# alshai/rowbowt

Hardware: AMD Instinct MI355X
Metric: reads/s (100 bp, count+locate) (higher is better)
Workload: dtype u32/u64

## Files before the change

### rowbowt_amd/csrc/k_runs.hip

```cpp
#include <type_traits>

#include "rbg_runs2_device.hpp"
#include "rbg_jump.h"

namespace rbg {
namespace {

struct PackedBits {
    const uint4 *__restrict__ cp;
    uint4 w;
    uint32_t widx, navail;
    uint64_t sr;
    __device__ __forceinline__ uint32_t next_word() {
        if (widx == 4) { w = *cp++; widx = 0; }
        const uint32_t v = w.x;
        w.x = w.y; w.y = w.z; w.z = w.w;
        ++widx;
        return v;
    }
    __device__ __forceinline__ uint32_t take(uint32_t nb) {
        if (navail < nb) { sr |= static_cast<uint64_t>(next_word()) << navail; navail += 32; }
        const uint32_t v = static_cast<uint32_t>(sr & ((uint64_t(1) << nb) - 1));
        sr >>= nb;
        navail -= nb;
        return v;
    }
};

struct JumpLoad {
    const uint4 *__restrict__ tab;
    __device__ __forceinline__ void operator()(uint64_t b, uint32_t s, uint32_t kw[4], uint32_t vw[4]) const {
        const uint4 *sl = tab + (4 * b + 2 * s);
        const uint4 k = sl[0], v = sl[1];
        kw[0] = k.x; kw[1] = k.y; kw[2] = k.z; kw[3] = k.w;
        vw[0] = v.x; vw[1] = v.y; vw[2] = v.z; vw[3] = v.w;
    }
};

template <typename P, bool TOEHOLD, bool PACKED = false, bool STATS = false, bool GLDS = false, bool STAGE = false>
__global__ __launch_bounds__(512, STATS ? 2 : 4) void k_find_range_runs(const DevIndex ix, const void *__restrict__ src_a,
                                                        const void *__restrict__ src_b, const uint64_t N,
                                                        uint64_t *__restrict__ lo_out, uint64_t *__restrict__ hi_out,
                                                        uint64_t *__restrict__ ss_out, unsigned long long *__restrict__ stats,
                                                        const uint32_t *__restrict__ sel, const uint32_t *__restrict__ nsel) {
    const uint64_t Neff = sel ? static_cast<uint64_t>(*nsel) : N;
    const uint8_t *__restrict__ seqs = static_cast<const uint8_t *>(src_a);
    const uint64_t *__restrict__ off = static_cast<const uint64_t *>(src_b);
    const uint4 *__restrict__ chunks = static_cast<const uint4 *>(src_a);
    const uint2 *__restrict__ meta = static_cast<const uint2 *>(src_b);
    __shared__ uint8_t s_lut[256];
    __shared__ uint8_t s_lut2[256];
    __shared__ uint8_t s_mslot[4];
    __shared__ __align__(16) unsigned char s_tile[GLDS ? 8 * kTileBytes : 16];
    __shared__ uint32_t s_codes[STAGE ? 8 * kStageWords * 64 : 1];
    for (int t = threadIdx.x; t < 256; t += blockDim.x) {
        s_lut[t] = ix.lut[t];
        s_lut2[t] = ix.nmajor ? ix.lut2[t] : 0xFFu;
    }
    RBG_RUN_SEARCH2_SHARED;
    const RunSearch2<P> S2 = stage_run_search2<P>(ix, s_tab_first, s_ent2, s_dir2, s_rec2, s_dyn);
    const uint32_t *tab_first = s_tab_first;
    lds_byte *tile = (lds_byte *)s_tile + (GLDS ? (threadIdx.x >> 6) * kTileBytes : 0u);
    if (PACKED || STAGE) {
        for (int t = threadIdx.x; t < 256; t += blockDim.x)
            if (s_lut2[t] != 0xFFu) s_mslot[s_lut2[t] & 3u] = s_lut[t];
        __syncthreads();
    }
    const uint32_t D = ix.run_ksteps, DMASK = ix.run_depth_mask | 1u;
    const uint32_t M = ix.nmajor;
    const uint32_t lane = threadIdx.x & (kWave - 1);
    lds_u32 *codes = (lds_u32 *)s_codes + (STAGE ? (threadIdx.x >> 6) * (kStageWords * 64u) + lane : 0u);
    const StageTab stage_tab{ix.stage_code[0], ix.stage_code[1], ix.stage_byte[0], ix.stage_byte[1], ix.stage_shift};
    const bool stage_on = STAGE && ix.stage_ok != 0 && M == 4;

    unsigned long long c_occ = 0, c_reads = 0;
    uint32_t c_matched = 0;
    unsigned long long st[kStatSearchN] = {0, 0, 0, 0, 0, 0, 0, 0};
    const uint64_t stride = static_cast<uint64_t>(gridDim.x) * blockDim.x;
    const uint64_t wave_first = static_cast<uint64_t>(blockIdx.x) * blockDim.x + (threadIdx.x & ~(kWave - 1));
    for (uint64_t base = wave_first; base < Neff; base += stride) {
        bool valid = base + lane < Neff;
        const uint64_t i = (sel && valid) ? static_cast<uint64_t>(sel[base + lane]) : base + lane;
        uint64_t beg = 0, p = 0;
        PackedBits bs{chunks, make_uint4(0, 0, 0, 0), 4u, 0u, 0ull};
        if (PACKED) {
            if (valid) {
                const uint2 mt = meta[i];
                if (mt.y & 0x80000000u) valid = false;
                else { p = mt.y; bs.cp = chunks + mt.x; }
            }
        } else if (valid) { beg = off[i]; p = off[i + 1]; }
        bool staged = false;
        if constexpr (STAGE && !PACKED) {
            if (stage_on && __ballot(valid && p - beg > kStageCap) == 0) {
                uint32_t nch = 0;
                const bool bad = valid && stage_read(reinterpret_cast<const uint4 *>(seqs), beg, p, stage_tab, codes, nch);
                if (STATS) st[kStChunks] += nch;
                staged = __ballot(bad) == 0;
                if (staged) { p -= beg; beg = 0; }
                else if (STATS) st[kStChunks] -= nch;
            }
        }
        auto walk = [&](auto staged_tag) __attribute__((always_inline)) {
            constexpr bool STAGED = decltype(staged_tag)::value;
            const uint64_t p_end = p;
            uint64_t p_min = p;
            const uint32_t m32 = static_cast<uint32_t>(p);
            uint64_t lo = 0, hi = ix.n - 1;
            uint64_t k = TOEHOLD ? ix.last_run_sample : 0;
            bool alive = valid;
            bool pend = false;
            uint32_t pend_d = 0, pend_rec = 0;
            uint64_t pend_e = 0;
            ByteCursor rd{reinterpret_cast<const uint4 *>(seqs), ~uint64_t(0), make_uint4(0, 0, 0, 0)};
            bool jumped = false;
            if constexpr (STAGED && sizeof(P) == 4) {
                if (valid && ix.jump && m32 >= ix.jump_k) {
                    JumpKey key{{codes[0], codes[64], codes[128], codes[192]}};
                    jump_key_mask(key, ix.jump_k);
                    uint32_t v[3] = {0, 0, 0}, nbk = 0;
                    if (jump_probe(JumpLoad{static_cast<const uint4 *>(ix.jump)}, ix.jump_buckets, key, v, nbk)) {
                        lo = v[0]; hi = v[1];
                        if (TOEHOLD) k = v[2] == 0xFFFFFFFFu ? ~uint64_t(0) : static_cast<uint64_t>(v[2]);
                        p -= ix.jump_k;
                        jumped = true;
                        if (STATS) st[kStSymbols] += ix.jump_k;
                    }
                    if (STATS) st[kStFtab] += nbk;
                }
            }
            if (!jumped && valid && ix.ftab_k && p - beg >= ix.ftab_k) {
                uint64_t idx = 0;
                bool all_major = true;
                PackedBits probe = bs;
                if constexpr (STAGED) {
                    const uint32_t w0 = codes[0];
                    idx = ix.ftab_k >= 16u ? w0 : (w0 & ((1u << (2u * ix.ftab_k)) - 1u));
                } else if (PACKED) {
                    idx = probe.take(2 * ix.ftab_k);
                } else {
                    uint64_t pw = 1;
                    for (uint32_t t = 1; t <= ix.ftab_k; ++t) {
                        const uint32_t mm = s_lut2[rd.at(p - t)];
                        all_major = all_major && mm != 0xFFu;
                        idx += (mm & 3u) * pw;
                        pw *= M;
                    }
                }
                uint64_t flo, fhi2, fk;
                if (STATS) { if (!STAGED) p_min = p - ix.ftab_k; if (all_major) st[kStFtab] += 1; }
                if (all_major && ftab_lookup<P>(ix, idx, flo, fhi2, fk)) {
                    if (PACKED) bs = probe;
                    lo = flo; hi = fhi2;
                    if (TOEHOLD) k = fk;
                    p -= ix.ftab_k;
                    if (STATS) st[kStSymbols] += ix.ftab_k;
                    if (hi < lo) { alive = false; p = beg; }
                }
            }
            struct Pick { uint32_t d, adv, rec; bool ok; };
            auto pick_at = [&](const uint64_t pp) __attribute__((always_inline)) -> Pick {
                Pick s{0u, 1u, 0u, true};
                if constexpr (STAGED) {
                    s.adv = pp < D ? static_cast<uint32_t>(pp) : D;
                    s.adv = 32u - static_cast<uint32_t>(__clz(DMASK & ((2u << (s.adv - 1)) - 1u)));
                    const uint32_t t0 = m32 - static_cast<uint32_t>(pp);
                    const lds_u32 *cw = codes + (t0 >> 4) * 64u;
                    const uint32_t v = __builtin_amdgcn_alignbit(cw[64], cw[0], (t0 & 15u) * 2u) & ((1u << (2u * s.adv)) - 1u);
                    s.rec = run_record(tab_first, s.adv, s.adv == 1 ? static_cast<uint32_t>(s_mslot[v]) : v);
                    s.d = s.adv - 1;
                } else if (PACKED) {
                    s.adv = pp < D ? static_cast<uint32_t>(pp) : D;
                    s.adv = 32u - static_cast<uint32_t>(__clz(DMASK & ((2u << (s.adv - 1)) - 1u)));
                    const uint32_t v = bs.take(2 * s.adv);
                    s.rec = run_record(tab_first, s.adv, s.adv == 1 ? static_cast<uint32_t>(s_mslot[v]) : v);
                    s.d = s.adv - 1;
                } else {
                    const uint64_t q = pp - 1;
                    const uint32_t c = rd.at(q);
                    if (STATS && q < p_min) p_min = q;
                    const uint32_t m0 = s_lut2[c];
                    uint32_t acc = m0;
                    if (m0 != 0xFFu) {
                        uint32_t pw = M, run_acc = m0;
    #pragma unroll 1
                        for (uint32_t t = 1; t < static_cast<uint32_t>(kMaxRunDepth); ++t) {
                            if (t >= D || q < beg + t) break;
                            const uint32_t mm = s_lut2[rd.at(q - t)];
                            if (STATS && q - t < p_min) p_min = q - t;
                            if (mm == 0xFFu) break;
                            run_acc += mm * pw;
                            pw *= M;
                            if ((DMASK >> t) & 1u) { s.adv = t + 1; acc = run_acc; }
                        }
                    }
                    if (s.adv == 1) {
                        const uint32_t slot = s_lut[c];
                        if (slot == 0xFFu || slot >= static_cast<uint32_t>(kLdsSyms)) s.ok = false;
                        else s.rec = run_record(tab_first, 1u, slot);
                    } else {
                        s.d = s.adv - 1;
                        s.rec = run_record(tab_first, s.adv, acc);
                    }
                }
                return s;
            };
            constexpr bool AHEAD = !PACKED || STAGED;
            Pick cur{0u, 1u, 0u, false};
            RunHot Rcur{0, 0};
            if (AHEAD && alive && p > beg) {
                cur = pick_at(p);
                if (cur.ok) Rcur = load_run_tab<P>(S2, cur.d, cur.rec);
            }
            while (__ballot(alive && p > beg)) {
                bool stepping = alive && p > beg;
                if (!AHEAD && stepping) {
                    cur = pick_at(p);
                    if (cur.ok) Rcur = load_run_tab<P>(S2, cur.d, cur.rec);
                }
                if (stepping && !cur.ok) { alive = false; stepping = false; }
                const uint32_t d = cur.d, adv = cur.adv, rec = cur.rec;
                const RunHot R = Rcur;
                const uint64_t p_next = p - adv;
                if (AHEAD && stepping && p_next > beg) {
                    cur = pick_at(p_next);
                    if (cur.ok) Rcur = load_run_tab<P>(S2, cur.d, cur.rec);
                }
                RunStep r;
                lane_lf2_quad<P, STATS, false, GLDS>(S2, stepping, d, rec, R, lo, hi + 1, r, st, tile);
                if (stepping) {
                    if (STATS) st[kStSymbols] += adv;
                    const uint64_t c_inside = r.c_upto - r.c_before;
                    if (c_inside == 0) {
                        alive = false;
                    } else {
                        if (TOEHOLD) {
                            if (r.inside) k = k - adv;
                            else { pend = true; pend_d = d; pend_rec = rec; pend_e = r.samp_e; k = 0; }
                        }
                        lo = r.F + r.c_before;
                        hi = lo + c_inside - 1;
                        p = p_next;
                    }
                }
            }
            if (TOEHOLD && alive && pend) {
                k += run_step_sample2<P>(ix, S2, pend_d, pend_rec, pend_e);
                if (STATS) st[kStResample] += 1;
            }
            if (STATS && !PACKED && !STAGED && p_end > p_min) st[kStChunks] += ((p_end - 1) >> 4) - (p_min >> 4) + 1;
            if (STATS && PACKED && valid) st[kStChunks] += (p_end + 63) >> 6;
            if (!alive) { lo = 1; hi = 0; k = 0; }
            if (valid) {
                lo_out[i] = lo;
                hi_out[i] = hi;
                if (TOEHOLD) ss_out[i] = k;
                c_reads += 1;
                if (alive) { c_matched += 1; c_occ += hi - lo + 1; }
            }
        };
        if (STAGE && staged) walk(std::integral_constant<bool, STAGE>{}); else walk(std::false_type{});
    }
    c_reads = wave_sum(c_reads);
    const unsigned long long w_matched = wave_sum(static_cast<unsigned long long>(c_matched));
    c_occ = wave_sum(c_occ);
    if (lane == 0 && c_reads) {
        atomicAdd(&ix.counters[0], c_reads);
        if (w_matched) atomicAdd(&ix.counters[1], w_matched);
        if (c_occ) atomicAdd(&ix.counters[2], c_occ);
    }
    if (STATS) {
#pragma unroll
        for (int t = 0; t < kStatSearchN; ++t) {
            const unsigned long long v = wave_sum(st[t]);
            if (lane == 0 && v) atomicAdd(&stats[t], v);
        }
    }
}

template <typename P> struct ChunkR { static constexpr int v = 8; };
__device__ __forceinline__ uint64_t locus_toehold_r(const DevIndex &ix, const uint64_t key, const uint64_t *__restrict__ k, const uint64_t i) {
    if (key == ~uint64_t(0)) return k[i];
    const uint32_t low = ix.order_lowbits, db = ix.order_dbits;
    const uint64_t doc = (key >> low) & ((uint64_t(1) << db) - 1u);
    return ix.order_docs[doc] + (((key >> (db + low)) << low) | (key & ((uint64_t(1) << low) - 1u)));
}

template <typename P, typename OUT = uint64_t, bool STATS = false, bool SUB = false, bool HI8 = false>
__global__ __launch_bounds__(256, 4) void k_locate_fill_runs2(const DevIndex ix, const uint64_t *__restrict__ lo,
                                                          const uint64_t *__restrict__ hi, const uint64_t *__restrict__ k,
                                                          const uint64_t N, const uint64_t max_hits,
                                                          const uint64_t *__restrict__ loc_off, OUT *__restrict__ locs,
                                                          const uint64_t *__restrict__ sub, const uint32_t *__restrict__ order,
                                                          const uint64_t *__restrict__ skeys, unsigned long long *__restrict__ stats) {
    constexpr int kChunkR = ChunkR<P>::v;
    constexpr bool RING = true;
    using Stage = ChainStage<P, kChunkR, SUB, RING, HI8>;
    __shared__ Stage S;
    const uint64_t out_elem0 = reinterpret_cast<uintptr_t>(locs) / sizeof(OUT);
    const int wv = threadIdx.x >> 6, lane = threadIdx.x & (kWave - 1);
    unsigned long long c_locs = 0;
    unsigned long long st_phi = 0, st_ent = 0, st_chains = 0;
    const uint64_t n = ix.n;
    const uint64_t stride = static_cast<uint64_t>(gridDim.x) * blockDim.x;
    for (uint64_t base = static_cast<uint64_t>(blockIdx.x) * blockDim.x + wv * kWave; base < N; base += stride) {
        const uint64_t j = base + lane;
        uint64_t i = j;
        if (order && j < N) i = order[j];
        uint64_t occ = 0, k1 = 0, dst = 0;
        if (i < N && j < N) {
            dst = loc_off[i];
            if (skeys) {
                if (ix.order_docs) k1 = locus_toehold_r(ix, skeys[j], k, i);
                else if (sizeof(P) == 4) { const uint32_t k32 = reinterpret_cast<const uint32_t *>(skeys)[j]; k1 = k32 == 0xFFFFFFFFu ? k[i] : k32; }
                else k1 = skeys[j];
                occ = loc_off[i + 1] - dst;
            } else {
                const uint64_t l = lo[i], h = hi[i];
                occ = h >= l ? h - l + 1 : 0;
                if (occ > max_hits) occ = max_hits;
                k1 = k[i];
            }
        }
        const uint64_t minus = (SUB && i < N && j < N) ? sub[i] : 0;
        const uint32_t a = (RING && occ) ? static_cast<uint32_t>((out_elem0 + dst) & static_cast<uint64_t>(kChunkR - 1)) : 0u;
        S.dst[wv][lane] = dst - a;
        if (SUB) S.minus[wv][lane] = minus;
        const bool off_text = Stage::kSentinel && k1 >= n;
        if (off_text && occ) locs[dst] = static_cast<OUT>(k1 - minus);
        c_locs += occ;
        if (STATS && occ) st_chains += 1;
        uint64_t wmax = occ + a;
#pragma unroll
        for (int o = kWave / 2; o > 0; o >>= 1) {
            const uint64_t other = __shfl_xor(wmax, o, kWave);
            wmax = other > wmax ? other : wmax;
        }
        for (uint64_t t0 = 0; t0 < wmax; t0 += kChunkR) {
            const uint32_t cnt = chain_round_count<kChunkR>(occ, t0);
            S.bounds[wv][lane] = chain_window_bounds<kChunkR>(occ, a, t0);
#pragma unroll 1
            for (int e = 0; e < kChunkR; ++e) {
                const bool mine = static_cast<uint32_t>(e) < cnt;
                if (mine && (e || t0)) {
                    uint64_t s;
                    if (k1 >= n) {
                        s = (ix.phi_last_base + (k1 - ix.phi_last_pos)) % n;
                    } else {
                        bool found;
                        uint64_t val;
                        uint32_t ents, rounds;
                        lane_phi<P>(ix, k1, found, val, ents, rounds);
                        if (STATS) { st_phi += 1; st_ent += ents + 7u * rounds; }
                        s = found ? val : ix.phi_last_base + k1 + 1;
                        if (s >= n) s -= n;
                    }
                    k1 = s;
                }
                if (mine) chain_put(S, wv, lane, a + static_cast<uint32_t>(t0) + e, k1, e == 0 && t0 == 0 && off_text);
            }
            wave_lds_sync();
            chain_flush(S, wv, lane, t0, locs);
            wave_lds_sync();
        }
        wave_lds_sync();
    }
    c_locs = wave_sum(c_locs);
    if (lane == 0 && c_locs) atomicAdd(&ix.counters[3], c_locs);
    if (STATS) {
        st_phi = wave_sum(st_phi);
        st_ent = wave_sum(st_ent);
        st_chains = wave_sum(st_chains);
        if (lane == 0) {
            if (st_phi) atomicAdd(&stats[kLsPhiSteps], st_phi);
            if (st_ent) atomicAdd(&stats[kLsPhiOvf], st_ent);
            if (st_chains) atomicAdd(&stats[kLsChains], st_chains);
            if (c_locs) atomicAdd(&stats[kLsLocs], c_locs);
        }
    }
}

}

int launch_find_range_runs_impl(const DevIndex &ix, const LaunchCfg &cfg, const void *src_a, const void *src_b, uint64_t N,
                                uint64_t *lo, uint64_t *hi, uint64_t *ssamp, void *stream, bool packed, unsigned long long *stats,
                                const uint32_t *sel = nullptr, const uint32_t *nsel = nullptr) {
    if (N == 0) return 0;
    hipStream_t st = static_cast<hipStream_t>(stream);
    const size_t lds = run_search2_lds(ix);
    static const bool glds = [] { const char *e = std::getenv("RBG_REC_FETCH"); return !(e && std::strcmp(e, "quad") == 0); }();
    static const bool stage = [] { const char *e = std::getenv("RBG_STAGE_READS"); return !(e && e[0] == '0'); }();
    LaunchCfg c = cfg;
    c.block_threads = 512;
    c.max_blocks = cfg.max_blocks > 0 ? std::max(1, cfg.max_blocks / 2) : 256 * 16;
    const dim3 grid(sel ? std::min(grid_for(c, N), 256) : grid_for(c, N)), block(512);
#define RBG_LAUNCH_FRR1(PT, TOE, PK, STS, GL, SG)                                                      \
    do {                                                                                               \
        auto kern = k_find_range_runs<PT, TOE, PK, STS, GL, SG>;                                       \
        raise_lds(kern, lds, (GL ? 8 * kTileBytes : 0) + (SG ? 8 * kStageWaveBytes : 0));             \
        hipLaunchKernelGGL(kern, grid, block, lds, st, ix, src_a, src_b, N, lo, hi, ssamp, stats, sel, nsel);     \
    } while (0)
#define RBG_LAUNCH_FRR(PT, TOE, PK, STS)                                                               \
    do {                                                                                               \
        if (glds && stage && !PK && !sel) RBG_LAUNCH_FRR1(PT, TOE, false, STS, true, true);            \
        else if (glds) RBG_LAUNCH_FRR1(PT, TOE, PK, STS, true, false);                                 \
        else RBG_LAUNCH_FRR1(PT, TOE, PK, STS, false, false);                                          \
    } while (0)
#define RBG_LAUNCH_FRR2(PT, TOE)                                                                       \
    do {                                                                                               \
        if (stats) { if (packed) return static_cast<int>(hipErrorNotSupported); RBG_LAUNCH_FRR(PT, TOE, false, true); } \
        else if (packed) RBG_LAUNCH_FRR(PT, TOE, true, false);                                         \
        else RBG_LAUNCH_FRR(PT, TOE, false, false);                                                    \
    } while (0)
    if (ix.pos_bytes == 4) {
        if (ssamp) RBG_LAUNCH_FRR2(uint32_t, true); else RBG_LAUNCH_FRR2(uint32_t, false);
    } else {
        if (ssamp) RBG_LAUNCH_FRR2(uint64_t, true); else RBG_LAUNCH_FRR2(uint64_t, false);
    }
#undef RBG_LAUNCH_FRR2
#undef RBG_LAUNCH_FRR
#undef RBG_LAUNCH_FRR1
    return static_cast<int>(hipGetLastError());
}

// ... 47 lines not shown
```

### rowbowt_amd/csrc/rbg_jump.h

```cpp
#pragma once

#include <cstdint>

#if defined(__HIPCC__)
#define RBG_JUMP_HD __host__ __device__ __forceinline__
#else
#define RBG_JUMP_HD inline
#endif

namespace rbg {

constexpr uint32_t kJumpMaxK = 64;
constexpr uint32_t kJumpMinK = 16;
constexpr uint32_t kJumpSlotWords = 8;
constexpr uint32_t kJumpBucketBytes = 64;
constexpr uint32_t kJumpEmptyTag = 0, kJumpFullTag = 1;
constexpr uint32_t kJumpDefaultK = 60;
constexpr uint64_t kJumpAutoMinBytes = uint64_t(256) << 20;

struct JumpKey {
    uint32_t w[4];
};

RBG_JUMP_HD void jump_key_mask(JumpKey &key, uint32_t K) {
    for (uint32_t i = 0; i < 4; ++i) {
        const uint32_t lo_sym = 16u * i;
        const uint32_t keep = K <= lo_sym ? 0u : (K - lo_sym >= 16u ? 16u : K - lo_sym);
        key.w[i] = keep == 16u ? key.w[i] : (key.w[i] & ((1u << (2u * keep)) - 1u));
    }
}

RBG_JUMP_HD void jump_key_set(JumpKey &key, uint32_t t, uint32_t c) {
    key.w[t >> 4] |= (c & 3u) << (2u * (t & 15u));
}

RBG_JUMP_HD uint64_t jump_hash(const JumpKey &key) {
    const uint64_t a = key.w[0] | (static_cast<uint64_t>(key.w[1]) << 32);
    const uint64_t b = key.w[2] | (static_cast<uint64_t>(key.w[3]) << 32);
    uint64_t h = (a * 0x9E3779B97F4A7C15ull) ^ ((b + 0x632BE59BD9B4E019ull) * 0xC2B2AE3D27D4EB4Full);
    h ^= h >> 29;
    h *= 0xBF58476D1CE4E5B9ull;
    h ^= h >> 32;
    return h;
}

RBG_JUMP_HD uint64_t jump_home(uint64_t h, uint64_t nb) {
    return ((h >> 32) * nb) >> 32;
}

template <typename Load>
RBG_JUMP_HD bool jump_probe(const Load &load, uint64_t nb, const JumpKey &key, uint32_t v[3], uint32_t &buckets) {
    uint64_t b = jump_home(jump_hash(key), nb);
    for (uint64_t step = 0; step < nb; ++step) {
        ++buckets;
        for (uint32_t s = 0; s < 2; ++s) {
            uint32_t kw[4], vw[4];
            load(b, s, kw, vw);
            if (vw[3] == kJumpEmptyTag) return false;
            if (kw[0] == key.w[0] && kw[1] == key.w[1] && kw[2] == key.w[2] && kw[3] == key.w[3]) {
                v[0] = vw[0]; v[1] = vw[1]; v[2] = vw[2];
                return true;
            }
        }
        b = b + 1 == nb ? 0 : b + 1;
    }
    return false;
}

inline uint64_t jump_buckets_for(uint64_t keys) { return keys ? keys : 1; }

}
```

### rowbowt_amd/csrc/rbg_runs2_device.hpp

```cpp
#pragma once

#include "rbg_runs_device.hpp"

namespace rbg {
namespace {

constexpr int kRunUniAt = 12;
constexpr uint32_t kLaneMaxZ = 15;
constexpr uint32_t kLanePhiMaxZ = 8;

template <typename P>
struct RunSearch2 {
    const uint64_t *hot;
    const uint64_t *ghot;
    const DevRunTab2 *gtab;
    const uint32_t *tab_first;
    const void *const *ent;
    const void *const *dir;
    const void *const *rec;
    const void *rec_any;
    uint32_t fill;
};

#define RBG_RUN_SEARCH2_SHARED                                            \
// ... 119 lines not shown
            A.feed(g, w0.x - a_lo, w0.y);
            A.feed(g + 1u, w0.z - a_lo, w0.w);
            A.feed(g + 2u, w1.x - a_lo, w1.y);
            A.feed(g + 3u, w1.z - a_lo, w1.w);
            if (B) {
                B->feed(g, w0.x - a_lo, w0.y);
                B->feed(g + 1u, w0.z - a_lo, w0.w);
                B->feed(g + 2u, w1.x - a_lo, w1.y);
                B->feed(g + 3u, w1.z - a_lo, w1.w);
            }
        }
        return;
    }
    u32x4a8 w[4], v[4];
#pragma unroll
    for (int j = 0; j < 4; ++j) {
        const uint32_t gj = 2u * j < zw ? 2u * j : zw;
        w[j] = *reinterpret_cast<const RBG_GLOBAL u32x4a8 *>(base + static_cast<uint64_t>(gj) * 8u);
    }
    const bool more = zw >= 8u;
    if (more) {
#pragma unroll
        for (int j = 0; j < 4; ++j) {
            const uint32_t gj = 8u + 2u * j < zw ? 8u + 2u * j : zw;
            v[j] = *reinterpret_cast<const RBG_GLOBAL u32x4a8 *>(base + static_cast<uint64_t>(gj) * 8u);
        }
    }
#pragma unroll
    for (int j = 0; j < 4; ++j) {
        A.feed(2u * j, w[j].x - a_lo, w[j].y);
        A.feed(2u * j + 1u, w[j].z - a_lo, w[j].w);
        if (B) {
            B->feed(2u * j, w[j].x - a_lo, w[j].y);
            B->feed(2u * j + 1u, w[j].z - a_lo, w[j].w);
        }
    }
    if (more) {
#pragma unroll
        for (int j = 0; j < 4; ++j) {
            A.feed(8u + 2u * j, v[j].x - a_lo, v[j].y);
            A.feed(8u + 2u * j + 1u, v[j].z - a_lo, v[j].w);
            if (B) {
                B->feed(8u + 2u * j, v[j].x - a_lo, v[j].y);
                B->feed(8u + 2u * j + 1u, v[j].z - a_lo, v[j].w);
            }
        }
    }
}

constexpr uint32_t kRecScanZ = 7u;
constexpr uint32_t kRecScanZ2 = 15u;
struct LaneRank {
    uint32_t c = 0, lo32 = 0, p = 0, z = 0;
    bool inside = false, pending = false;
    uint32_t qa = 0, a_lo = 0;
};
__device__ __forceinline__ uint32_t sub_sat(const uint32_t a, const uint32_t b) { return __builtin_elementwise_sub_sat(a, b); }
struct LaneRec {
    uint32_t w[16];
    __device__ __forceinline__ void load(const void *__restrict__ recs, const uint64_t at) {
        const RBG_GLOBAL u32x4 *p = as_global<u32x4>(static_cast<const void *>(static_cast<const char *>(recs) + at * 64u));
        const u32x4 a = p[0], b = p[1], c = p[2], d = p[3];
        w[0] = a.x; w[1] = a.y; w[2] = a.z; w[3] = a.w; w[4] = b.x; w[5] = b.y; w[6] = b.z; w[7] = b.w;
        w[8] = c.x; w[9] = c.y; w[10] = c.z; w[11] = c.w; w[12] = d.x; w[13] = d.y; w[14] = d.z; w[15] = d.w;
    }
    __device__ __forceinline__ bool compact() const { return (w[2] & kRec2Compact) != 0; }
    __device__ __forceinline__ void pivots(const uint32_t a_lo, const uint32_t qa, LaneRank &out) const {
        out.qa = qa; out.a_lo = a_lo;
        const uint32_t z = w[3], stride = (z + 12u) / 13u;
        uint32_t m = 0;
#pragma unroll
        for (uint32_t j = 0; j < kRec2Pivots; ++j) m += ((j + 1u) * stride < z && w[4 + j] - a_lo < qa) ? 1u : 0u;
        const uint32_t adv = m * stride;
        out.p = w[0] + adv;
        out.z = (z - adv) < stride ? (z - adv) : stride;
        out.pending = true;
    }
    template <bool NEED_C>
    __device__ __forceinline__ void rank1(const uint32_t sh, const uint32_t a_lo, const uint32_t qa, const uint32_t o, LaneRank &out) const {
        out.qa = qa; out.a_lo = a_lo; out.p = w[0]; out.pending = false;
        const uint32_t mask = ~(~0u << (sh & 31u));
        const uint32_t s0 = w[4] - a_lo, d0 = qa - s0, om1 = o - 1u;
        const bool b0 = (w[2] & 15u) != 0u && s0 < qa;
        uint32_t add = b0 ? (d0 < w[5] ? d0 : w[5]) : 0u, c = b0 ? 1u : 0u;
        bool ins = b0 && d0 <= w[5];
#pragma unroll
        for (uint32_t k = 0; k < kRec2CompactIn; ++k) {
            const uint32_t v = w[6 + k], off = v & mask, len = v >> (sh & 31u);
            const uint32_t d = sub_sat(o, off);
            add += d < len ? d : len;
            if (NEED_C) { c += off < o ? 1u : 0u; ins = ins || (om1 - off) < len; }
        }
        out.c = NEED_C ? c : 1u; out.lo32 = w[3] + add; out.inside = ins;
    }
    __device__ __forceinline__ void rank2(const uint32_t sh, const uint32_t a_lo, const uint32_t qa0, const uint32_t o0, const uint32_t qa1, const uint32_t o1,
                                          LaneRank &A, LaneRank &B) const {
        A.qa = qa0; A.a_lo = a_lo; A.p = w[0]; A.pending = false;
        B.qa = qa1; B.a_lo = a_lo; B.p = w[0]; B.pending = false;
        const uint32_t mask = ~(~0u << (sh & 31u));
        const uint32_t s0 = w[4] - a_lo, l0 = w[5], da = qa0 - s0, db = qa1 - s0, om1 = o1 - 1u;
        const bool have = (w[2] & 15u) != 0u, ba = have && s0 < qa0, bb = have && s0 < qa1;
        uint32_t add_a = ba ? (da < l0 ? da : l0) : 0u, add_b = bb ? (db < l0 ? db : l0) : 0u, c = bb ? 1u : 0u;
        bool ins = bb && db <= l0;
#pragma unroll
        for (uint32_t k = 0; k < kRec2CompactIn; ++k) {
            const uint32_t v = w[6 + k], off = v & mask, len = v >> (sh & 31u);
            const uint32_t ea = sub_sat(o0, off), eb = sub_sat(o1, off);
            add_a += ea < len ? ea : len;
            add_b += eb < len ? eb : len;
            c += off < o1 ? 1u : 0u;
            ins = ins || (om1 - off) < len;
        }
        A.c = 1u;
        A.lo32 = w[3] + add_a; A.inside = false;
        B.c = c; B.lo32 = w[3] + add_b; B.inside = ins;
    }
};

template <typename P, bool WIDE = true>
__device__ __forceinline__ void lane_finish(const RunSearch2<P> &S, const uint32_t d, const uint32_t rec, LaneRank &A, LaneRank *B, uint32_t &rounds, uint32_t &ents) {
    const bool pb = B && B->pending;
    if (!(A.pending || pb)) return;
    const char *__restrict__ tent = static_cast<const char *>(S.ent[d]) + run_first<P>(S, rec) * 8u;
    constexpr uint32_t kMaxZ = WIDE ? kRecScanZ2 : kRecScanZ;
    if (A.pending && A.z > kMaxZ) lane_narrow(tent, A.a_lo, A.qa, A.p, A.z, kMaxZ, 8u, rounds);
    if (pb && B->z > kMaxZ) lane_narrow(tent, B->a_lo, B->qa, B->p, B->z, kMaxZ, 8u, rounds);
    u32x4a8 wa[4], wb[4];
    if (A.pending) {
        const RBG_GLOBAL char *base = as_global<char>(static_cast<const void *>(tent)) + static_cast<uint64_t>(A.p) * 8u;
#pragma unroll
        for (int j = 0; j < 4; ++j) wa[j] = *reinterpret_cast<const RBG_GLOBAL u32x4a8 *>(base + static_cast<uint64_t>(2u * j < A.z ? 2u * j : A.z) * 8u);
    }
    if (pb) {
        const RBG_GLOBAL char *base = as_global<char>(static_cast<const void *>(tent)) + static_cast<uint64_t>(B->p) * 8u;
#pragma unroll
        for (int j = 0; j < 4; ++j) wb[j] = *reinterpret_cast<const RBG_GLOBAL u32x4a8 *>(base + static_cast<uint64_t>(2u * j < B->z ? 2u * j : B->z) * 8u);
    }
    auto take = [&](LaneRank &R, const u32x4a8 (&w)[4]) {
        LaneQ Q;
        Q.qa = R.qa; Q.zlim = R.z;
#pragma unroll
        for (int j = 0; j < 4; ++j) {
            Q.feed(2u * j, w[j].x - R.a_lo, w[j].y);
            Q.feed(2u * j + 1u, w[j].z - R.a_lo, w[j].w);
        }
        if (WIDE && R.z > kRecScanZ && Q.pb) {
            const RBG_GLOBAL char *base = as_global<char>(static_cast<const void *>(tent)) + static_cast<uint64_t>(R.p) * 8u;
            u32x4a8 v[4];
#pragma unroll
            for (int j = 0; j < 4; ++j) v[j] = *reinterpret_cast<const RBG_GLOBAL u32x4a8 *>(base + static_cast<uint64_t>(8u + 2u * j < R.z ? 8u + 2u * j : R.z) * 8u);
#pragma unroll
            for (int j = 0; j < 4; ++j) {
                Q.feed(8u + 2u * j, v[j].x - R.a_lo, v[j].y);
                Q.feed(8u + 2u * j + 1u, v[j].z - R.a_lo, v[j].w);
            }
            ents += 8u;
        }
        R.c = Q.c;
        const uint32_t dd = Q.qa - Q.ks, len = Q.kn - Q.kc;
        R.lo32 = Q.c ? Q.kc + (dd < len ? dd : len) : Q.fc;
        R.inside = Q.c != 0u && dd <= len;
        ents += (R.z < 8u ? R.z + 1u : 8u);
    };
    if (A.pending) take(A, wa);
    if (pb) take(*B, wb);
}


template <typename P, bool STATS = false, bool LEAN = false>
__device__ __forceinline__ void lane_lf2_tab(const RunSearch2<P> &S, const uint32_t d, const uint32_t rec, const RunHot &R, const uint64_t q0, const uint64_t q1, RunStep &out,
                                             unsigned long long *st = nullptr) {
    constexpr bool W = sizeof(P) == 8;
    out.F = 0;
    const uint32_t sh = R.dir_shift;
    const uint64_t b0 = pos_bucket<P>(q0, sh), b1 = pos_bucket<P>(q1, sh);
    if (const void *__restrict__ recs = S.rec[d]) {
        const uint32_t al0 = W ? pos_bucket_base32(q0, sh) - (1u << S.fill) : 0u;
        const uint32_t al1 = W ? pos_bucket_base32(q1, sh) - (1u << S.fill) : 0u;
        const uint32_t qa0 = static_cast<uint32_t>(q0) - al0, qa1 = static_cast<uint32_t>(q1) - al1;
        const uint32_t o0 = pos_bucket_offset(q0, sh), o1 = pos_bucket_offset(q1, sh);
        LaneRank A, B;
        uint32_t h0, h1;
        uint32_t rounds = 0, ents = 0;
        LaneRec r0;
        r0.load(recs, R.dir_off + b0);
        h0 = h1 = r0.w[1];
        if (b1 == b0) {
            if (r0.compact()) r0.rank2(sh, al0, qa0, o0, qa1, o1, A, B);
            else { r0.pivots(al0, qa0, A); r0.pivots(al1, qa1, B); }
            lane_finish<P, !LEAN>(S, d, rec, A, &B, rounds, ents);
        } else if constexpr (LEAN) {
            if (r0.compact()) r0.template rank1<false>(sh, al0, qa0, o0, A); else r0.pivots(al0, qa0, A);
            lane_finish<P, !LEAN>(S, d, rec, A, nullptr, rounds, ents);
            r0.load(recs, R.dir_off + b1);
            h1 = r0.w[1];
            if (r0.compact()) r0.template rank1<true>(sh, al1, qa1, o1, B); else r0.pivots(al1, qa1, B);
            lane_finish<P, !LEAN>(S, d, rec, B, nullptr, rounds, ents);
        } else {
            LaneRec r1;
            r1.load(recs, R.dir_off + b1);
            h1 = r1.w[1];
            if (r0.compact()) r0.template rank1<false>(sh, al0, qa0, o0, A); else r0.pivots(al0, qa0, A);
            if (r1.compact()) r1.template rank1<true>(sh, al1, qa1, o1, B); else r1.pivots(al1, qa1, B);
            lane_finish<P, !LEAN>(S, d, rec, A, &B, rounds, ents);
        }
        if (STATS) { st[kStSlots] += b1 != b0 ? 2 : 1; st[kStSearch] += rounds; st[kStDense] += ents; st[kStSteps] += 1; }
        const uint64_t y0 = static_cast<uint64_t>(h0) << 31, y1 = static_cast<uint64_t>(h1) << 31;
        out.c_before = W ? y0 + static_cast<uint32_t>(A.lo32 - static_cast<uint32_t>(y0)) : A.lo32;
        out.c_upto = W ? y1 + static_cast<uint32_t>(B.lo32 - static_cast<uint32_t>(y1)) : B.lo32;
        out.inside = B.c != 0 && B.inside;
        out.samp_e = static_cast<uint64_t>(B.p) + B.c - 1u;
        return;
    }
    const char *__restrict__ tent = static_cast<const char *>(S.ent[d]) + run_first<P>(S, rec) * 8u;
    const void *__restrict__ dir = S.dir[d];
    uint32_t a0, h0, e0, a1, h1, e1;
    load_dir2<P>(dir, R.dir_off + b0, a0, h0, e0);
    a1 = a0; h1 = h0; e1 = e0;
    if (b1 != b0) load_dir2<P>(dir, R.dir_off + b1, a1, h1, e1);
    if (STATS) st[kStSlots] += b1 != b0 ? 2 : 1;
    uint32_t p0 = a0 ? a0 - 1u : 0u, z0 = e0 - p0;
    uint32_t p1 = a1 ? a1 - 1u : 0u, z1 = e1 - p1;
    const uint32_t al0 = W ? pos_bucket_base32(q0, sh) - (1u << S.fill) : 0u;
    const uint32_t al1 = W ? pos_bucket_base32(q1, sh) - (1u << S.fill) : 0u;
    const uint32_t qa0 = static_cast<uint32_t>(q0) - al0, qa1 = static_cast<uint32_t>(q1) - al1;
    uint32_t rounds = 0;
    if (z0 > kLaneMaxZ) lane_narrow(tent, al0, qa0, p0, z0, kLaneMaxZ, 8u, rounds);
    if (z1 > kLaneMaxZ) lane_narrow(tent, al1, qa1, p1, z1, kLaneMaxZ, 8u, rounds);
    if (STATS) st[kStSearch] += rounds;
    const bool shared = p1 + z1 <= p0 + kLaneMaxZ && (!W || b1 - b0 <= 1u);
    LaneQ A, B;
    A.qa = qa0; A.zlim = z0;
    if (shared) {
        B.qa = static_cast<uint32_t>(q1) - al0; B.zlim = p1 + z1 - p0;
        const uint32_t zw = B.zlim > z0 ? B.zlim : z0;
        lane_scan<LEAN>(tent, p0, zw, al0, A, &B);
        if (STATS) st[kStDense] += zw + 1u;
        p1 = p0;
    } else {
        B.qa = qa1; B.zlim = z1;
        lane_scan<LEAN>(tent, p0, z0, al0, A, nullptr);
        lane_scan<LEAN>(tent, p1, z1, al1, B, nullptr);
        if (STATS) st[kStDense] += z0 + z1 + 2u;
    }
    bool inside = false;
    uint32_t lo32a = A.fc, lo32b = B.fc;
    if (A.c) {
        const uint32_t dd = A.qa - A.ks, len = A.kn - A.kc;
        lo32a = A.kc + (dd < len ? dd : len);
    }
    if (B.c) {
        const uint32_t dd = B.qa - B.ks, len = B.kn - B.kc;
        lo32b = B.kc + (dd < len ? dd : len);
        inside = dd <= len;
    }
    const uint64_t y0 = static_cast<uint64_t>(h0) << 31, y1 = static_cast<uint64_t>(h1) << 31;
    out.c_before = W ? y0 + static_cast<uint32_t>(lo32a - static_cast<uint32_t>(y0)) : lo32a;
    out.c_upto = W ? y1 + static_cast<uint32_t>(lo32b - static_cast<uint32_t>(y1)) : lo32b;
    out.inside = inside;
    out.samp_e = static_cast<uint64_t>(p1) + B.c - 1u;
    if (STATS) st[kStSteps] += 1;
}

template <typename P, bool STATS = false, bool LEAN = false>
__device__ __forceinline__ void lane_lf2(const RunSearch2<P> &S, const uint32_t d, const uint32_t rec, const uint64_t q0, const uint64_t q1, RunStep &out,
                                         unsigned long long *st = nullptr) {
    const RunHot R = load_run_tab<P>(S, d, rec);
    lane_lf2_tab<P, STATS, LEAN>(S, d, rec, R, q0, q1, out, st);
}

__device__ __forceinline__ uint32_t quad_xor1(const uint32_t v) { return static_cast<uint32_t>(__builtin_amdgcn_mov_dpp(static_cast<int>(v), 0xB1, 0xF, 0xF, true)); }
__device__ __forceinline__ uint32_t quad_xor2(const uint32_t v) { return static_cast<uint32_t>(__builtin_amdgcn_mov_dpp(static_cast<int>(v), 0x4E, 0xF, 0xF, true)); }
template <int C>
__device__ __forceinline__ uint32_t quad_bcast(const uint32_t v) { return static_cast<uint32_t>(__builtin_amdgcn_mov_dpp(static_cast<int>(v), C * 0x55, 0xF, 0xF, true)); }
__device__ __forceinline__ void quad_transpose16(uint32_t (&w)[16], const uint32_t p) {
    const bool p0 = (p & 1u) != 0u, p1 = (p & 2u) != 0u;
#pragma unroll
    for (int b = 0; b < 4; b += 2)
#pragma unroll
        for (int k = 0; k < 4; ++k) {
            const uint32_t lo = w[4 * b + k], hi = w[4 * (b + 1) + k];
            const uint32_t t = quad_xor1(p0 ? lo : hi);
            w[4 * b + k] = p0 ? t : lo;
            w[4 * (b + 1) + k] = p0 ? hi : t;
        }
#pragma unroll
    for (int b = 0; b < 2; ++b)
#pragma unroll
        for (int k = 0; k < 4; ++k) {
            const uint32_t lo = w[4 * b + k], hi = w[4 * (b + 2) + k];
            const uint32_t t = quad_xor2(p1 ? lo : hi);
            w[4 * b + k] = p1 ? t : lo;
            w[4 * (b + 2) + k] = p1 ? hi : t;
        }
}
constexpr uint32_t kTileRound = 1024u + 16u;
constexpr uint32_t kTileBytes = 4u * kTileRound;
typedef __attribute__((address_space(3))) unsigned char lds_byte;
template <int r>
__device__ __forceinline__ void glds_round(const uint32_t a_lo, const uint32_t a_hi, const uint32_t p, lds_byte *tile) {
    const uint64_t an = (static_cast<uint64_t>(quad_bcast<r>(a_hi)) << 32) | quad_bcast<r>(a_lo);
    __builtin_amdgcn_global_load_lds(reinterpret_cast<const RBG_GLOBAL void *>(an + 16u * p), reinterpret_cast<__attribute__((address_space(3))) void *>(tile + r * kTileRound), 16, 0, 0);
}
template <typename P, bool STATS = false, bool LEAN = false, bool GLDS = false>
__device__ __forceinline__ void lane_lf2_quad(const RunSearch2<P> &S, const bool stepping, const uint32_t d, const uint32_t rec, const RunHot &R, const uint64_t q0,
                                              const uint64_t q1, RunStep &out, unsigned long long *st = nullptr, lds_byte *tile = nullptr) {
    constexpr bool W = sizeof(P) == 8;
    const uint32_t sh = R.dir_shift;
    const bool by_rec = stepping && S.rec[d] != nullptr;
    if (stepping && !by_rec) lane_lf2_tab<P, STATS, LEAN>(S, d, rec, R, q0, q1, out, st);
    if (__ballot(by_rec) == 0) return;
    const uint32_t p = threadIdx.x & 3u;
    const uint64_t b0 = by_rec ? pos_bucket<P>(q0, sh) : 0u, b1 = by_rec ? pos_bucket<P>(q1, sh) : 0u;
    const char *recs = static_cast<const char *>(by_rec ? S.rec[d] : S.rec_any);
    const uint64_t a0 = reinterpret_cast<uint64_t>(recs) + (by_rec ? (R.dir_off + b0) * 64u : 0u);
    const uint32_t a_lo = static_cast<uint32_t>(a0), a_hi = static_cast<uint32_t>(a0 >> 32);
    LaneRec r0, r1;
    uint32_t (&w0)[16] = r0.w;
    const bool two = by_rec && b1 != b0;
    if constexpr (GLDS) {
        glds_round<0>(a_lo, a_hi, p, tile);
        glds_round<1>(a_lo, a_hi, p, tile);
        glds_round<2>(a_lo, a_hi, p, tile);
        glds_round<3>(a_lo, a_hi, p, tile);
        if constexpr (!LEAN) { if (two) r1.load(recs, R.dir_off + b1); }
        asm volatile("s_waitcnt vmcnt(0)" ::: "memory");
        const lds_byte *own = tile + (threadIdx.x & 3u) * kTileRound + (threadIdx.x & 60u) * 16u;
        typedef __attribute__((address_space(3))) const u32x4 lds_u32x4;
        const u32x4 t0 = reinterpret_cast<lds_u32x4 *>(own)[0], t1 = reinterpret_cast<lds_u32x4 *>(own)[1], t2 = reinterpret_cast<lds_u32x4 *>(own)[2],
                    t3 = reinterpret_cast<lds_u32x4 *>(own)[3];
        w0[0] = t0.x; w0[1] = t0.y; w0[2] = t0.z; w0[3] = t0.w; w0[4] = t1.x; w0[5] = t1.y; w0[6] = t1.z; w0[7] = t1.w;
        w0[8] = t2.x; w0[9] = t2.y; w0[10] = t2.z; w0[11] = t2.w; w0[12] = t3.x; w0[13] = t3.y; w0[14] = t3.z; w0[15] = t3.w;
        asm volatile("s_waitcnt lgkmcnt(0)" ::: "memory");
    } else {
#define RBG_QUAD_ROUND(r)                                                                                                             \
    {                                                                                                                                  \
        const uint64_t an = (static_cast<uint64_t>(quad_bcast<r>(a_hi)) << 32) | quad_bcast<r>(a_lo);                                  \
        const u32x4 t = *as_global<u32x4>(reinterpret_cast<const void *>(an + 16u * p));                                                \
        w0[4 * r] = t.x; w0[4 * r + 1] = t.y; w0[4 * r + 2] = t.z; w0[4 * r + 3] = t.w;                                                  \
    }
        RBG_QUAD_ROUND(0) RBG_QUAD_ROUND(1) RBG_QUAD_ROUND(2) RBG_QUAD_ROUND(3)
#undef RBG_QUAD_ROUND
        if constexpr (!LEAN) { if (two) r1.load(recs, R.dir_off + b1); }
        quad_transpose16(w0, p);
    }
    if (!by_rec) return;
    out.F = 0;
    const uint32_t al0 = W ? pos_bucket_base32(q0, sh) - (1u << S.fill) : 0u;
    const uint32_t al1 = W ? pos_bucket_base32(q1, sh) - (1u << S.fill) : 0u;
    const uint32_t qa0 = static_cast<uint32_t>(q0) - al0, qa1 = static_cast<uint32_t>(q1) - al1;
    const uint32_t o0 = pos_bucket_offset(q0, sh), o1 = pos_bucket_offset(q1, sh);
    LaneRank A, B;
    uint32_t h0 = w0[1], h1 = w0[1], rounds = 0, ents = 0;
    if (!two) {
        if (r0.compact()) r0.rank2(sh, al0, qa0, o0, qa1, o1, A, B);
        else { r0.pivots(al0, qa0, A); r0.pivots(al1, qa1, B); }
        lane_finish<P, !LEAN>(S, d, rec, A, &B, rounds, ents);
    } else if constexpr (LEAN) {
        if (r0.compact()) r0.template rank1<false>(sh, al0, qa0, o0, A); else r0.pivots(al0, qa0, A);
        lane_finish<P, !LEAN>(S, d, rec, A, nullptr, rounds, ents);
        r0.load(recs, R.dir_off + b1);
        h1 = w0[1];
        if (r0.compact()) r0.template rank1<true>(sh, al1, qa1, o1, B); else r0.pivots(al1, qa1, B);
        lane_finish<P, !LEAN>(S, d, rec, B, nullptr, rounds, ents);
    } else {
        h1 = r1.w[1];
        if (r0.compact()) r0.template rank1<false>(sh, al0, qa0, o0, A); else r0.pivots(al0, qa0, A);
        if (r1.compact()) r1.template rank1<true>(sh, al1, qa1, o1, B); else r1.pivots(al1, qa1, B);
        lane_finish<P, !LEAN>(S, d, rec, A, &B, rounds, ents);
    }
    if (STATS) { st[kStSlots] += two ? 2 : 1; st[kStSearch] += rounds; st[kStDense] += ents; st[kStSteps] += 1; }
    const uint64_t y0 = static_cast<uint64_t>(h0) << 31, y1 = static_cast<uint64_t>(h1) << 31;
    out.c_before = W ? y0 + static_cast<uint32_t>(A.lo32 - static_cast<uint32_t>(y0)) : A.lo32;
    out.c_upto = W ? y1 + static_cast<uint32_t>(B.lo32 - static_cast<uint32_t>(y1)) : B.lo32;
    out.inside = B.c != 0 && B.inside;
    out.samp_e = static_cast<uint64_t>(B.p) + B.c - 1u;
}
template <typename P, bool STATS = false, bool LEAN = false>
__device__ __forceinline__ void lane_lf2_quad(const RunSearch2<P> &S, const bool stepping, const uint32_t d, const uint32_t rec, const uint64_t q0, const uint64_t q1,
                                              RunStep &out, unsigned long long *st = nullptr) {
    const RunHot R = load_run_tab<P>(S, stepping ? d : 0u, stepping ? rec : 0u);
    lane_lf2_quad<P, STATS, LEAN, false>(S, stepping, d, rec, R, q0, q1, out, st, nullptr);
}

template <typename P>
__device__ __forceinline__ uint64_t run_step_sample2(const DevIndex &ix, const RunSearch2<P> &S, const uint32_t d, const uint32_t rec, const uint64_t rel) {
    return RunList<P>::samp(ix.run_samp[d], run_first<P>(S, rec) + rel);
}

template <typename P>
__device__ __forceinline__ void lane_phi(const DevIndex &ix, const uint64_t q, bool &found, uint64_t &val, uint32_t &ents, uint32_t &rounds) {
    constexpr bool W = sizeof(P) == 8;
    constexpr uint32_t EB = W ? 12u : 8u;
    const uint32_t sh = ix.phi_dir_shift;
    const uint64_t b = q >> sh;
    const u32x2a4 dw = *reinterpret_cast<const RBG_GLOBAL u32x2a4 *>(as_global<uint32_t>(ix.phi_dir) + b);
    uint64_t g0;
    uint32_t inb = dw.y - dw.x;
    if constexpr (W) {
        const uint64_t s0 = as_global<uint64_t>(ix.phi_super)[b >> ix.phi_super_shift];
        g0 = s0 + static_cast<uint32_t>(dw.x - static_cast<uint32_t>(s0));
    } else {
        g0 = dw.x;
    }
    const uint64_t pred = g0 ? g0 - 1u : 0u;
    uint32_t z = inb + (g0 ? 1u : 0u);
    const uint32_t a_lo = W ? static_cast<uint32_t>(b << sh) - (1u << ix.run_fill_shift) : 0u;
    const uint32_t qa = static_cast<uint32_t>(q) - a_lo;
    const char *__restrict__ tent = static_cast<const char *>(ix.phi_ent) + pred * EB;
    uint32_t p = 0;
    rounds = 0;
    if (z > kLanePhiMaxZ) lane_narrow(tent, a_lo, qa, p, z, kLanePhiMaxZ, EB, rounds);
    ents = z;
    const RBG_GLOBAL char *base = as_global<char>(static_cast<const void *>(tent)) + static_cast<uint64_t>(p) * EB;
    uint32_t c = 0, ks = 0, kb_lo = 0, kb_hi = 0;
    const uint32_t zl = z ? z - 1u : 0u;
    const bool more = z > 4u;
    if constexpr (W) {
        u32x3a4 w[4], v[4];
#pragma unroll
        for (int j = 0; j < 4; ++j) w[j] = *reinterpret_cast<const RBG_GLOBAL u32x3a4 *>(base + static_cast<uint64_t>(static_cast<uint32_t>(j) < zl ? static_cast<uint32_t>(j) : zl) * 12u);
        if (more) {
#pragma unroll
            for (int j = 0; j < 4; ++j) v[j] = *reinterpret_cast<const RBG_GLOBAL u32x3a4 *>(base + static_cast<uint64_t>(4u + j < zl ? 4u + j : zl) * 12u);
        }
#pragma unroll
        for (int j = 0; j < 4; ++j) {
            const uint32_t sa = w[j].x - a_lo;
            const bool nb = static_cast<uint32_t>(j) < z && sa < qa;
            ks = nb ? sa : ks; kb_lo = nb ? w[j].y : kb_lo; kb_hi = nb ? w[j].z : kb_hi;
            c += nb ? 1u : 0u;
        }
        if (more) {
#pragma unroll
            for (int j = 0; j < 4; ++j) {
                const uint32_t sa = v[j].x - a_lo;
                const bool nb = 4u + j < z && sa < qa;
                ks = nb ? sa : ks; kb_lo = nb ? v[j].y : kb_lo; kb_hi = nb ? v[j].z : kb_hi;
                c += nb ? 1u : 0u;
            }
        }
    } else {
        u32x4a8 w[2], v[2];
#pragma unroll
        for (int j = 0; j < 2; ++j) w[j] = *reinterpret_cast<const RBG_GLOBAL u32x4a8 *>(base + static_cast<uint64_t>(2u * j < zl ? 2u * j : zl) * 8u);
        if (more) {
#pragma unroll
            for (int j = 0; j < 2; ++j) v[j] = *reinterpret_cast<const RBG_GLOBAL u32x4a8 *>(base + static_cast<uint64_t>(4u + 2u * j < zl ? 4u + 2u * j : zl) * 8u);
        }
#pragma unroll
        for (int j = 0; j < 2; ++j) {
            const bool nb0 = 2u * j < z && w[j].x < qa;
            ks = nb0 ? w[j].x : ks; kb_lo = nb0 ? w[j].y : kb_lo;
            const bool nb1 = 2u * j + 1u < z && w[j].z < qa;
            ks = nb1 ? w[j].z : ks; kb_lo = nb1 ? w[j].w : kb_lo;
            c += (nb0 ? 1u : 0u) + (nb1 ? 1u : 0u);
        }
        if (more) {
#pragma unroll
            for (int j = 0; j < 2; ++j) {
                const bool nb0 = 4u + 2u * j < z && v[j].x < qa;
                ks = nb0 ? v[j].x : ks; kb_lo = nb0 ? v[j].y : kb_lo;
                const bool nb1 = 4u + 2u * j + 1u < z && v[j].z < qa;
                ks = nb1 ? v[j].z : ks; kb_lo = nb1 ? v[j].w : kb_lo;
                c += (nb0 ? 1u : 0u) + (nb1 ? 1u : 0u);
            }
        }
    }
    found = c != 0;
    val = ((static_cast<uint64_t>(kb_hi) << 32) | kb_lo) + static_cast<uint32_t>(qa - ks);
}

}
}
```

Measured before the change: 1.995 billion.

## Probe jump hash table with wave-cooperative quad loads

Measured after the change: 2.082 billion, median of 6. 1.04x the previous value.

```diff
diff --git a/rowbowt_amd/csrc/k_runs.hip b/rowbowt_amd/csrc/k_runs.hip
--- a/rowbowt_amd/csrc/k_runs.hip
+++ b/rowbowt_amd/csrc/k_runs.hip
@@ -27,15 +27,26 @@
     }
 };
 
-struct JumpLoad {
-    const uint4 *__restrict__ tab;
-    __device__ __forceinline__ void operator()(uint64_t b, uint32_t s, uint32_t kw[4], uint32_t vw[4]) const {
-        const uint4 *sl = tab + (4 * b + 2 * s);
-        const uint4 k = sl[0], v = sl[1];
-        kw[0] = k.x; kw[1] = k.y; kw[2] = k.z; kw[3] = k.w;
-        vw[0] = v.x; vw[1] = v.y; vw[2] = v.z; vw[3] = v.w;
-    }
-};
+template <bool GLDS>
+__device__ __forceinline__ bool jump_probe_wave(const void *__restrict__ tab, const uint64_t nb, const bool probing, const JumpKey &key, uint32_t v[3],
+                                                uint32_t &buckets, lds_byte *tile) {
+    uint32_t state = probing ? kJumpNext : kJumpAbsent;
+    uint64_t b = probing ? jump_home(jump_hash(key), nb) : 0u;
+    uint64_t left = nb;
+    while (__ballot(state == kJumpNext)) {
+        const bool undecided = state == kJumpNext;
+        uint32_t w[16];
+        quad_fetch_issue<GLDS>(reinterpret_cast<uint64_t>(tab) + (undecided ? b : 0u) * kJumpBucketBytes, w, tile);
+        quad_fetch_take<GLDS>(w, tile);
+        if (undecided) {
+            ++buckets;
+            state = jump_bucket(w, key, v);
+            b = jump_next(b, nb);
+            if (--left == 0 && state == kJumpNext) state = kJumpAbsent;
+        }
+    }
+    return state <= kJumpHit1;
+}
 
 template <typename P, bool TOEHOLD, bool PACKED = false, bool STATS = false, bool GLDS = false, bool STAGE = false>
 __global__ __launch_bounds__(512, STATS ? 2 : 4) void k_find_range_runs(const DevIndex ix, const void *__restrict__ src_a,
@@ -115,11 +126,12 @@
             ByteCursor rd{reinterpret_cast<const uint4 *>(seqs), ~uint64_t(0), make_uint4(0, 0, 0, 0)};
             bool jumped = false;
             if constexpr (STAGED && sizeof(P) == 4) {
-                if (valid && ix.jump && m32 >= ix.jump_k) {
+                if (ix.jump) {
+                    const bool probing = valid && m32 >= ix.jump_k;
                     JumpKey key{{codes[0], codes[64], codes[128], codes[192]}};
                     jump_key_mask(key, ix.jump_k);
                     uint32_t v[3] = {0, 0, 0}, nbk = 0;
-                    if (jump_probe(JumpLoad{static_cast<const uint4 *>(ix.jump)}, ix.jump_buckets, key, v, nbk)) {
+                    if (jump_probe_wave<GLDS>(ix.jump, ix.jump_buckets, probing, key, v, nbk, tile)) {
                         lo = v[0]; hi = v[1];
                         if (TOEHOLD) k = v[2] == 0xFFFFFFFFu ? ~uint64_t(0) : static_cast<uint64_t>(v[2]);
                         p -= ix.jump_k;
diff --git a/rowbowt_amd/csrc/rbg_jump.h b/rowbowt_amd/csrc/rbg_jump.h
--- a/rowbowt_amd/csrc/rbg_jump.h
+++ b/rowbowt_amd/csrc/rbg_jump.h
@@ -48,21 +48,32 @@
     return ((h >> 32) * nb) >> 32;
 }
 
+constexpr uint32_t kJumpHit0 = 0, kJumpHit1 = 1, kJumpAbsent = 2, kJumpNext = 3;
+RBG_JUMP_HD uint32_t jump_bucket(const uint32_t w[16], const JumpKey &key, uint32_t v[3]) {
+    for (uint32_t s = 0; s < 2; ++s) {
+        const uint32_t *sl = w + kJumpSlotWords * s;
+        if (sl[7] == kJumpEmptyTag) return kJumpAbsent;
+        if (sl[0] == key.w[0] && sl[1] == key.w[1] && sl[2] == key.w[2] && sl[3] == key.w[3]) {
+            v[0] = sl[4]; v[1] = sl[5]; v[2] = sl[6];
+            return s;
+        }
+    }
+    return kJumpNext;
+}
+
+RBG_JUMP_HD uint64_t jump_next(uint64_t b, uint64_t nb) { return b + 1 == nb ? 0 : b + 1; }
+
 template <typename Load>
 RBG_JUMP_HD bool jump_probe(const Load &load, uint64_t nb, const JumpKey &key, uint32_t v[3], uint32_t &buckets) {
     uint64_t b = jump_home(jump_hash(key), nb);
     for (uint64_t step = 0; step < nb; ++step) {
         ++buckets;
-        for (uint32_t s = 0; s < 2; ++s) {
-            uint32_t kw[4], vw[4];
-            load(b, s, kw, vw);
-            if (vw[3] == kJumpEmptyTag) return false;
-            if (kw[0] == key.w[0] && kw[1] == key.w[1] && kw[2] == key.w[2] && kw[3] == key.w[3]) {
-                v[0] = vw[0]; v[1] = vw[1]; v[2] = vw[2];
-                return true;
-            }
-        }
-        b = b + 1 == nb ? 0 : b + 1;
+        uint32_t w[16];
+        load(b, 0, w, w + 4);
+        load(b, 1, w + 8, w + 12);
+        const uint32_t r = jump_bucket(w, key, v);
+        if (r != kJumpNext) return r != kJumpAbsent;
+        b = jump_next(b, nb);
     }
     return false;
 }
diff --git a/rowbowt_amd/csrc/rbg_runs2_device.hpp b/rowbowt_amd/csrc/rbg_runs2_device.hpp
--- a/rowbowt_amd/csrc/rbg_runs2_device.hpp
+++ b/rowbowt_amd/csrc/rbg_runs2_device.hpp
@@ -445,6 +445,41 @@
     const uint64_t an = (static_cast<uint64_t>(quad_bcast<r>(a_hi)) << 32) | quad_bcast<r>(a_lo);
     __builtin_amdgcn_global_load_lds(reinterpret_cast<const RBG_GLOBAL void *>(an + 16u * p), reinterpret_cast<__attribute__((address_space(3))) void *>(tile + r * kTileRound), 16, 0, 0);
 }
+template <bool GLDS>
+__device__ __forceinline__ void quad_fetch_issue(const uint64_t a0, uint32_t (&w)[16], lds_byte *tile) {
+    const uint32_t p = threadIdx.x & 3u;
+    const uint32_t a_lo = static_cast<uint32_t>(a0), a_hi = static_cast<uint32_t>(a0 >> 32);
+    if constexpr (GLDS) {
+        glds_round<0>(a_lo, a_hi, p, tile);
+        glds_round<1>(a_lo, a_hi, p, tile);
+        glds_round<2>(a_lo, a_hi, p, tile);
+        glds_round<3>(a_lo, a_hi, p, tile);
+    } else {
+#define RBG_QUAD_ROUND(r)                                                                                                             \
+    {                                                                                                                                  \
+        const uint64_t an = (static_cast<uint64_t>(quad_bcast<r>(a_hi)) << 32) | quad_bcast<r>(a_lo);                                  \
+        const u32x4 t = *as_global<u32x4>(reinterpret_cast<const void *>(an + 16u * p));                                                \
+        w[4 * r] = t.x; w[4 * r + 1] = t.y; w[4 * r + 2] = t.z; w[4 * r + 3] = t.w;                                                      \
+    }
+        RBG_QUAD_ROUND(0) RBG_QUAD_ROUND(1) RBG_QUAD_ROUND(2) RBG_QUAD_ROUND(3)
+#undef RBG_QUAD_ROUND
+    }
+}
+template <bool GLDS>
+__device__ __forceinline__ void quad_fetch_take(uint32_t (&w)[16], lds_byte *tile) {
+    if constexpr (GLDS) {
+        asm volatile("s_waitcnt vmcnt(0)" ::: "memory");
+        const lds_byte *own = tile + (threadIdx.x & 3u) * kTileRound + (threadIdx.x & 60u) * 16u;
+        typedef __attribute__((address_space(3))) const u32x4 lds_u32x4;
+        const u32x4 t0 = reinterpret_cast<lds_u32x4 *>(own)[0], t1 = reinterpret_cast<lds_u32x4 *>(own)[1], t2 = reinterpret_cast<lds_u32x4 *>(own)[2],
+                    t3 = reinterpret_cast<lds_u32x4 *>(own)[3];
+        w[0] = t0.x; w[1] = t0.y; w[2] = t0.z; w[3] = t0.w; w[4] = t1.x; w[5] = t1.y; w[6] = t1.z; w[7] = t1.w;
+        w[8] = t2.x; w[9] = t2.y; w[10] = t2.z; w[11] = t2.w; w[12] = t3.x; w[13] = t3.y; w[14] = t3.z; w[15] = t3.w;
+        asm volatile("s_waitcnt lgkmcnt(0)" ::: "memory");
+    } else {
+        quad_transpose16(w, threadIdx.x & 3u);
+    }
+}
 template <typename P, bool STATS = false, bool LEAN = false, bool GLDS = false>
 __device__ __forceinline__ void lane_lf2_quad(const RunSearch2<P> &S, const bool stepping, const uint32_t d, const uint32_t rec, const RunHot &R, const uint64_t q0,
                                               const uint64_t q1, RunStep &out, unsigned long long *st = nullptr, lds_byte *tile = nullptr) {
@@ -453,40 +488,15 @@
     const bool by_rec = stepping && S.rec[d] != nullptr;
     if (stepping && !by_rec) lane_lf2_tab<P, STATS, LEAN>(S, d, rec, R, q0, q1, out, st);
     if (__ballot(by_rec) == 0) return;
-    const uint32_t p = threadIdx.x & 3u;
     const uint64_t b0 = by_rec ? pos_bucket<P>(q0, sh) : 0u, b1 = by_rec ? pos_bucket<P>(q1, sh) : 0u;
     const char *recs = static_cast<const char *>(by_rec ? S.rec[d] : S.rec_any);
     const uint64_t a0 = reinterpret_cast<uint64_t>(recs) + (by_rec ? (R.dir_off + b0) * 64u : 0u);
-    const uint32_t a_lo = static_cast<uint32_t>(a0), a_hi = static_cast<uint32_t>(a0 >> 32);
     LaneRec r0, r1;
     uint32_t (&w0)[16] = r0.w;
     const bool two = by_rec && b1 != b0;
-    if constexpr (GLDS) {
-        glds_round<0>(a_lo, a_hi, p, tile);
-        glds_round<1>(a_lo, a_hi, p, tile);
-        glds_round<2>(a_lo, a_hi, p, tile);
-        glds_round<3>(a_lo, a_hi, p, tile);
-        if constexpr (!LEAN) { if (two) r1.load(recs, R.dir_off + b1); }
-        asm volatile("s_waitcnt vmcnt(0)" ::: "memory");
-        const lds_byte *own = tile + (threadIdx.x & 3u) * kTileRound + (threadIdx.x & 60u) * 16u;
-        typedef __attribute__((address_space(3))) const u32x4 lds_u32x4;
-        const u32x4 t0 = reinterpret_cast<lds_u32x4 *>(own)[0], t1 = reinterpret_cast<lds_u32x4 *>(own)[1], t2 = reinterpret_cast<lds_u32x4 *>(own)[2],
-                    t3 = reinterpret_cast<lds_u32x4 *>(own)[3];
-        w0[0] = t0.x; w0[1] = t0.y; w0[2] = t0.z; w0[3] = t0.w; w0[4] = t1.x; w0[5] = t1.y; w0[6] = t1.z; w0[7] = t1.w;
-        w0[8] = t2.x; w0[9] = t2.y; w0[10] = t2.z; w0[11] = t2.w; w0[12] = t3.x; w0[13] = t3.y; w0[14] = t3.z; w0[15] = t3.w;
-        asm volatile("s_waitcnt lgkmcnt(0)" ::: "memory");
-    } else {
-#define RBG_QUAD_ROUND(r)                                                                                                             \
-    {                                                                                                                                  \
-        const uint64_t an = (static_cast<uint64_t>(quad_bcast<r>(a_hi)) << 32) | quad_bcast<r>(a_lo);                                  \
-        const u32x4 t = *as_global<u32x4>(reinterpret_cast<const void *>(an + 16u * p));                                                \
-        w0[4 * r] = t.x; w0[4 * r + 1] = t.y; w0[4 * r + 2] = t.z; w0[4 * r + 3] = t.w;                                                  \
-    }
-        RBG_QUAD_ROUND(0) RBG_QUAD_ROUND(1) RBG_QUAD_ROUND(2) RBG_QUAD_ROUND(3)
-#undef RBG_QUAD_ROUND
-        if constexpr (!LEAN) { if (two) r1.load(recs, R.dir_off + b1); }
-        quad_transpose16(w0, p);
-    }
+    quad_fetch_issue<GLDS>(a0, w0, tile);
+    if constexpr (!LEAN) { if (two) r1.load(recs, R.dir_off + b1); }
+    quad_fetch_take<GLDS>(w0, tile);
     if (!by_rec) return;
     out.F = 0;
     const uint32_t al0 = W ? pos_bucket_base32(q0, sh) - (1u << S.fill) : 0u;
```
